# sebrahimi1988/dss-ml-at-scale

Measured on AMD Instinct MI355X. Metric: samples/sec, higher is better.
Workload: dtype bf16; 1 GPU; model=resnet18, global_batch=212, parallelism=dp1+hipgraph

## Files before the change

### mi355x_scale/models/resnet.py

```python
from __future__ import annotations

from typing import List, Optional, Type, Union

import torch
import torch.nn as nn

from ..ops.conv3x3 import Conv3x3
from ..ops.fused_bn import FusedBNReLU2d
from ..ops.maxpool import MaxPool3x3s2
from ..ops.stemconv import StemConv2d


def _conv3x3(cin: int, cout: int, stride: int = 1) -> nn.Conv2d:
    if stride == 1 and cin == cout:
        return Conv3x3(cin, cout)
    return nn.Conv2d(cin, cout, 3, stride=stride, padding=1, bias=False)


def _conv1x1(cin: int, cout: int, stride: int = 1) -> nn.Conv2d:
    return nn.Conv2d(cin, cout, 1, stride=stride, bias=False)


class BasicBlock(nn.Module):
    expansion = 1

    def __init__(self, cin: int, cout: int, stride: int = 1,
                 downsample: Optional[nn.Module] = None):
        super().__init__()
        self.conv1 = _conv3x3(cin, cout, stride)
        self.bn1 = FusedBNReLU2d(cout)
        self.conv2 = _conv3x3(cout, cout)
        self.bn2 = FusedBNReLU2d(cout)
        self.downsample = downsample

    def forward(self, x: torch.Tensor) -> torch.Tensor:
        identity = x if self.downsample is None else self.downsample(x)
        out = self.bn1(self.conv1(x))
        return self.bn2(self.conv2(out), residual=identity)


class Bottleneck(nn.Module):
    expansion = 4

    def __init__(self, cin: int, cout: int, stride: int = 1,
                 downsample: Optional[nn.Module] = None):
        super().__init__()
        self.conv1 = _conv1x1(cin, cout)
        self.bn1 = FusedBNReLU2d(cout)
        self.conv2 = _conv3x3(cout, cout, stride)
        self.bn2 = FusedBNReLU2d(cout)
        self.conv3 = _conv1x1(cout, cout * self.expansion)
        self.bn3 = FusedBNReLU2d(cout * self.expansion)
        self.downsample = downsample

    def forward(self, x: torch.Tensor) -> torch.Tensor:
        identity = x if self.downsample is None else self.downsample(x)
        out = self.bn1(self.conv1(x))
        out = self.bn2(self.conv2(out))
        return self.bn3(self.conv3(out), residual=identity)


class ResNet(nn.Module):
    def __init__(self, block: Type[Union[BasicBlock, Bottleneck]],
                 layers: List[int], num_classes: int = 1000,
                 zero_init_residual: bool = True):
        super().__init__()
        self.inplanes = 64
        self.conv1 = StemConv2d()
        self.bn1 = FusedBNReLU2d(64)
        self.maxpool = MaxPool3x3s2()
        self.layer1 = self._make_layer(block, 64, layers[0])
        self.layer2 = self._make_layer(block, 128, layers[1], stride=2)
        self.layer3 = self._make_layer(block, 256, layers[2], stride=2)
        self.layer4 = self._make_layer(block, 512, layers[3], stride=2)
        self.avgpool = nn.AdaptiveAvgPool2d(1)
        self.fc = nn.Linear(512 * block.expansion, num_classes)

        for m in self.modules():
            if isinstance(m, nn.Conv2d):
                nn.init.kaiming_normal_(m.weight, mode="fan_out",
                                        nonlinearity="relu")
            elif isinstance(m, nn.BatchNorm2d):
                nn.init.ones_(m.weight)
                nn.init.zeros_(m.bias)
        if zero_init_residual:
            for m in self.modules():
                if isinstance(m, Bottleneck):
                    nn.init.zeros_(m.bn3.weight)
                elif isinstance(m, BasicBlock):
                    nn.init.zeros_(m.bn2.weight)

    def _make_layer(self, block, planes: int, blocks: int,
                    stride: int = 1) -> nn.Sequential:
        downsample = None
        if stride != 1 or self.inplanes != planes * block.expansion:
            downsample = nn.Sequential(
                _conv1x1(self.inplanes, planes * block.expansion, stride),
                FusedBNReLU2d(planes * block.expansion, relu=False),
            )
        layers = [block(self.inplanes, planes, stride, downsample)]
        self.inplanes = planes * block.expansion
        layers += [block(self.inplanes, planes) for _ in range(1, blocks)]
        return nn.Sequential(*layers)

    def forward(self, x: torch.Tensor) -> torch.Tensor:
        if self.bn1.training and self.conv1.stats_ok(x):
            x, partial = self.conv1.forward_with_stats(x)
            x = self.bn1.forward_pooled(x, partial)
        else:
            x = self.bn1.forward_pooled(self.conv1(x))
        x = self.layer4(self.layer3(self.layer2(self.layer1(x))))
        x = self.avgpool(x).flatten(1)
        return self.fc(x)


def resnet18(num_classes: int = 1000) -> ResNet:
    return ResNet(BasicBlock, [2, 2, 2, 2], num_classes)


def resnet34(num_classes: int = 1000) -> ResNet:
    return ResNet(BasicBlock, [3, 4, 6, 3], num_classes)


def resnet50(num_classes: int = 1000) -> ResNet:
    return ResNet(Bottleneck, [3, 4, 6, 3], num_classes)


MODELS = {"resnet18": resnet18, "resnet34": resnet34, "resnet50": resnet50}


def build_model(name: str, num_classes: int = 1000) -> ResNet:
    try:
        return MODELS[name](num_classes)
    except KeyError:
        raise ValueError(f"unknown model {name!r}; have {sorted(MODELS)}")
```

### mi355x_scale/ops/csrc/bindings.cpp

```cpp

#include <torch/extension.h>
#include <ATen/hip/HIPContext.h>
#include <hip/hip_runtime.h>

extern "C" void launch_normalize_u8_to_bf16(
    const uint8_t* in, void* out, const float* scale_dev,
    const float* shift_dev, long long n, hipStream_t stream);

void normalize_u8_to_bf16(torch::Tensor in, torch::Tensor out,
                          torch::Tensor scale, torch::Tensor shift) {
  TORCH_CHECK(in.is_cuda() && out.is_cuda(), "tensors must be on GPU");
  TORCH_CHECK(in.scalar_type() == torch::kUInt8, "input must be uint8");
  TORCH_CHECK(out.scalar_type() == torch::kBFloat16, "output must be bf16");
  TORCH_CHECK(in.is_contiguous(), "input must be contiguous (NHWC)");
  TORCH_CHECK(in.numel() == out.numel(), "element count mismatch");
  TORCH_CHECK(scale.is_cuda() && shift.is_cuda() && scale.numel() == 3 &&
                  shift.numel() == 3,
              "scale/shift must be 3-element device float tensors");
  TORCH_CHECK(scale.scalar_type() == torch::kFloat32 &&
              shift.scalar_type() == torch::kFloat32,
              "scale/shift must be float32");
  auto stream = at::cuda::getCurrentHIPStream();
  launch_normalize_u8_to_bf16(
      in.data_ptr<uint8_t>(), out.data_ptr(),
// ... 81 lines not shown

void groupfit_final(torch::Tensor yT, torch::Tensor xc0, torch::Tensor xc1,
                    torch::Tensor xc2, torch::Tensor pj0, torch::Tensor pj1,
                    torch::Tensor pj2, torch::Tensor best_order,
                    torch::Tensor fitted, torch::Tensor params,
                    torch::Tensor status,
                    torch::Tensor b0, torch::Tensor b1, torch::Tensor b2,
                    torch::Tensor w0, torch::Tensor w1, torch::Tensor w2) {
  _check_f32(yT, "yT"); _check_f32(fitted, "fitted");
  _check_f32(params, "params");
  TORCH_CHECK(best_order.scalar_type() == torch::kInt32 &&
              best_order.is_cuda());
  int T = yT.size(0);
  long long G = yT.size(1);
  TORCH_CHECK(fitted.size(0) == T && fitted.size(1) == G);
  auto stream = at::cuda::getCurrentHIPStream();
  auto fp = [](torch::Tensor& t) -> const float* {
    return t.numel() ? t.data_ptr<float>() : nullptr;
  };
  launch_groupfit_final(
      yT.data_ptr<float>(), xc0.data_ptr<float>(), xc1.data_ptr<float>(),
      xc2.data_ptr<float>(), pj0.data_ptr<float>(), pj1.data_ptr<float>(),
      pj2.data_ptr<float>(), best_order.data_ptr<int>(),
      fitted.data_ptr<float>(), params.data_ptr<float>(),
      status.data_ptr<uint8_t>(),
      fp(b0), fp(b1), fp(b2), fp(w0), fp(w1), fp(w2),
      T, G, (int)xc0.size(1), stream.stream());
}

void diff_center(torch::Tensor yT, torch::Tensor wc, torch::Tensor wm,
                 int64_t S, int64_t d) {
  _check_f32(yT, "yT"); _check_f32(wc, "wc"); _check_f32(wm, "wm");
  auto stream = at::cuda::getCurrentHIPStream();
  launch_diff_center(yT.data_ptr<float>(), wc.data_ptr<float>(),
                     wm.data_ptr<float>(), yT.size(0), yT.size(1),
                     (int)S, (int)d, stream.stream());
}

void exog_project_mfma(torch::Tensor P, torch::Tensor wc,
                       torch::Tensor beta) {
  _check_f32(P, "P"); _check_f32(wc, "wc"); _check_f32(beta, "beta");
  TORCH_CHECK(P.size(1) == wc.size(0), "K mismatch");
  TORCH_CHECK(beta.size(0) == P.size(0) && beta.size(1) == wc.size(1));
  TORCH_CHECK(P.size(0) <= 16, "KX must fit one MFMA row tile");
  auto stream = at::cuda::getCurrentHIPStream();
  launch_exog_project_mfma(P.data_ptr<float>(), wc.data_ptr<float>(),
                           beta.data_ptr<float>(), P.size(1), wc.size(1),
                           P.size(0), stream.stream());
}


extern "C" int bn_reduce_blocks(long long rows, int C);
extern "C" void launch_bn_fwd_reduce(const void* x, float* partial,
                                     int nblocks, long long rows, int C,
                                     hipStream_t stream);
extern "C" void launch_bn_fwd_finalize(const float* partial, int nblocks,
                                       float* mean, float* invstd,
                                       float* running_mean,
                                       float* running_var, float momentum,
                                       float eps, long long rows, int C,
                                       int update_running,
                                       long long* num_batches_tracked,
                                       hipStream_t stream);
extern "C" void launch_bn_pool_bwd_reduce(
    const void* dp, const unsigned char* code, const void* x,
    const float* mean, const float* invstd, const float* weight,
    const float* bias, float* partial, int nblocks, int N, int H, int W,
    int Ho, int Wo, int C, hipStream_t stream);
extern "C" void launch_bn_pool_bwd_apply(
    const void* dp, const unsigned char* code, const void* x,
    const float* mean, const float* invstd, const float* bias,
    const float* k, void* dx, int N, int H, int W, int Ho, int Wo, int C,
    hipStream_t stream);
extern "C" void launch_bn_fwd_apply(const void* x, const void* res, void* y,
                                    const float* mean, const float* invstd,
                                    const float* weight, const float* bias,
                                    long long rows, int C, int relu,
                                    hipStream_t stream);
extern "C" void launch_bn_bwd_reduce(const void* dz, const void* y,
                                     const void* x, const float* mean,
                                     const float* invstd, float* partial,
                                     void* dym, int nblocks, long long rows,
                                     int C, int relu, hipStream_t stream);
extern "C" void launch_bn_bwd_reduce_rm(const void* dz, const void* x,
                                        const float* mean,
                                        const float* invstd,
                                        const float* weight,
                                        const float* bias, float* partial,
                                        void* dym, int nblocks,
                                        long long rows, int C,
                                        hipStream_t stream);
extern "C" void launch_bn_bwd_apply_rm(const void* dz, const void* x,
                                       const float* mean,
                                       const float* invstd,
                                       const float* bias, const float* k,
                                       void* dx, long long rows, int C,
                                       hipStream_t stream);
extern "C" void launch_bn_bwd_apply_dym(const void* dym, const void* x,
                                        const float* mean,
                                        const float* invstd, const float* k,
                                        void* dx, long long rows, int C,
                                        hipStream_t stream);
extern "C" void launch_bn_bwd_finalize(const float* partial, int nblocks,
                                       const float* invstd,
                                       const float* weight, float* dweight,
                                       float* dbias, float* k, long long rows,
                                       int C, int accumulate,
                                       hipStream_t stream);
extern "C" void launch_bn_bwd_apply(const void* dz, const void* y,
                                    const void* x, const float* mean,
                                    const float* invstd, const float* k,
                                    void* dx, void* dres, long long rows,
                                    int C, int relu, hipStream_t stream);

static void _check_bn_act(const torch::Tensor& t, const char* name) {
  TORCH_CHECK(t.is_cuda() && t.scalar_type() == torch::kBFloat16,
              name, " must be bf16 on GPU");
}

static long long _bn_rows(const torch::Tensor& x, int64_t C) {
  TORCH_CHECK(C % 8 == 0 && 256 % (C / 8) == 0,
              "C must be 8*2^k and <= 2048, got ", C);
  TORCH_CHECK(x.numel() % C == 0, "numel not divisible by C");
  return (long long)(x.numel() / C);
}

torch::Tensor bn_fwd_reduce(torch::Tensor x, int64_t C) {
  _check_bn_act(x, "x");
  long long rows = _bn_rows(x, C);
  int nb = bn_reduce_blocks(rows, (int)C);
  auto partial = torch::empty(
      {(int64_t)nb * 2 * C},
      torch::TensorOptions().dtype(torch::kFloat32).device(x.device()));
  launch_bn_fwd_reduce(x.data_ptr(), partial.data_ptr<float>(), nb, rows,
                       (int)C, at::cuda::getCurrentHIPStream().stream());
  return partial;
}

void bn_fwd_finalize(torch::Tensor partial, torch::Tensor mean,
                     torch::Tensor invstd, torch::Tensor running_mean,
                     torch::Tensor running_var, double momentum, double eps,
                     int64_t rows, int64_t C, bool update_running,
                     c10::optional<torch::Tensor> num_batches_tracked) {
  _check_f32(partial, "partial"); _check_f32(mean, "mean");
  _check_f32(invstd, "invstd");
  _check_f32(running_mean, "running_mean");
  _check_f32(running_var, "running_var");
  TORCH_CHECK(partial.numel() % (2 * C) == 0, "partial must be [nb*2C]");
  int nb = (int)(partial.numel() / (2 * C));
  long long* nbt_p = nullptr;
  if (num_batches_tracked.has_value()) {
    const torch::Tensor& nbt = *num_batches_tracked;
    TORCH_CHECK(nbt.is_cuda() && nbt.scalar_type() == torch::kInt64 &&
                    nbt.numel() == 1,
                "num_batches_tracked must be a 1-element int64 GPU tensor");
    nbt_p = reinterpret_cast<long long*>(nbt.data_ptr<int64_t>());
  }
  launch_bn_fwd_finalize(partial.data_ptr<float>(), nb,
                         mean.data_ptr<float>(), invstd.data_ptr<float>(),
                         running_mean.data_ptr<float>(),
                         running_var.data_ptr<float>(), (float)momentum,
                         (float)eps, rows, (int)C, update_running ? 1 : 0,
                         nbt_p, at::cuda::getCurrentHIPStream().stream());
}

void bn_fwd_apply(torch::Tensor x, torch::Tensor res, torch::Tensor y,
                  torch::Tensor mean, torch::Tensor invstd,
                  torch::Tensor weight, torch::Tensor bias, int64_t C,
                  bool relu) {
  _check_bn_act(x, "x"); _check_bn_act(y, "y");
  _check_f32(mean, "mean"); _check_f32(invstd, "invstd");
  _check_f32(weight, "weight"); _check_f32(bias, "bias");
  const void* res_p = nullptr;
  if (res.defined() && res.numel()) {
    _check_bn_act(res, "res");
    TORCH_CHECK(res.numel() == x.numel(), "residual shape mismatch");
    res_p = res.data_ptr();
  }
  launch_bn_fwd_apply(x.data_ptr(), res_p, y.data_ptr(),
                      mean.data_ptr<float>(), invstd.data_ptr<float>(),
                      weight.data_ptr<float>(), bias.data_ptr<float>(),
                      _bn_rows(x, C), (int)C, relu ? 1 : 0,
                      at::cuda::getCurrentHIPStream().stream());
}

torch::Tensor bn_bwd_reduce(torch::Tensor dz, torch::Tensor y,
                            torch::Tensor x, torch::Tensor mean,
                            torch::Tensor invstd, torch::Tensor dym,
                            int64_t C, bool relu) {
  _check_bn_act(dz, "dz"); _check_bn_act(y, "y"); _check_bn_act(x, "x");
  void* dym_p = nullptr;
  if (dym.defined() && dym.numel()) {
    _check_bn_act(dym, "dym");
    TORCH_CHECK(dym.numel() == x.numel(), "dym shape mismatch");
    dym_p = dym.data_ptr();
  }
  long long rows = _bn_rows(x, C);
  int nb = bn_reduce_blocks(rows, (int)C);
  auto partial = torch::empty(
      {(int64_t)nb * 2 * C},
      torch::TensorOptions().dtype(torch::kFloat32).device(x.device()));
  launch_bn_bwd_reduce(dz.data_ptr(), y.data_ptr(), x.data_ptr(),
                       mean.data_ptr<float>(), invstd.data_ptr<float>(),
                       partial.data_ptr<float>(), dym_p, nb, rows, (int)C,
                       relu ? 1 : 0,
                       at::cuda::getCurrentHIPStream().stream());
  return partial;
}

torch::Tensor bn_bwd_reduce_rm(torch::Tensor dz, torch::Tensor x,
                               torch::Tensor mean, torch::Tensor invstd,
                               torch::Tensor weight, torch::Tensor bias,
                               torch::Tensor dym, int64_t C) {
  _check_bn_act(dz, "dz"); _check_bn_act(x, "x");
  _check_f32(mean, "mean"); _check_f32(invstd, "invstd");
  _check_f32(weight, "weight"); _check_f32(bias, "bias");
  void* dym_p = nullptr;
  if (dym.defined() && dym.numel()) {
    _check_bn_act(dym, "dym");
    TORCH_CHECK(dym.numel() == x.numel(), "dym shape mismatch");
    dym_p = dym.data_ptr();
  }
  long long rows = _bn_rows(x, C);
  int nb = bn_reduce_blocks(rows, (int)C);
  auto partial = torch::empty(
      {(int64_t)nb * 2 * C},
      torch::TensorOptions().dtype(torch::kFloat32).device(x.device()));
  launch_bn_bwd_reduce_rm(dz.data_ptr(), x.data_ptr(),
                          mean.data_ptr<float>(), invstd.data_ptr<float>(),
                          weight.data_ptr<float>(), bias.data_ptr<float>(),
                          partial.data_ptr<float>(), dym_p, nb, rows,
                          (int)C, at::cuda::getCurrentHIPStream().stream());
  return partial;
}

void bn_bwd_apply_rm(torch::Tensor dz, torch::Tensor x, torch::Tensor mean,
                     torch::Tensor invstd, torch::Tensor bias,
                     torch::Tensor k, torch::Tensor dx, int64_t C) {
  _check_bn_act(dz, "dz"); _check_bn_act(x, "x"); _check_bn_act(dx, "dx");
  _check_f32(mean, "mean"); _check_f32(invstd, "invstd");
  _check_f32(bias, "bias"); _check_f32(k, "k");
  launch_bn_bwd_apply_rm(dz.data_ptr(), x.data_ptr(),
                         mean.data_ptr<float>(), invstd.data_ptr<float>(),
                         bias.data_ptr<float>(), k.data_ptr<float>(),
                         dx.data_ptr(), _bn_rows(x, C), (int)C,
                         at::cuda::getCurrentHIPStream().stream());
}

void bn_bwd_apply_dym(torch::Tensor dym, torch::Tensor x,
                      torch::Tensor mean, torch::Tensor invstd,
                      torch::Tensor k, torch::Tensor dx, int64_t C) {
  _check_bn_act(dym, "dym"); _check_bn_act(x, "x"); _check_bn_act(dx, "dx");
  _check_f32(mean, "mean"); _check_f32(invstd, "invstd");
  _check_f32(k, "k");
  launch_bn_bwd_apply_dym(dym.data_ptr(), x.data_ptr(),
                          mean.data_ptr<float>(), invstd.data_ptr<float>(),
                          k.data_ptr<float>(), dx.data_ptr(),
                          _bn_rows(x, C), (int)C,
                          at::cuda::getCurrentHIPStream().stream());
}

void bn_bwd_finalize(torch::Tensor partial, torch::Tensor invstd,
                     torch::Tensor weight, torch::Tensor dweight,
                     torch::Tensor dbias, torch::Tensor k, int64_t rows,
                     int64_t C, bool accumulate) {
  _check_f32(partial, "partial"); _check_f32(invstd, "invstd");
  _check_f32(weight, "weight"); _check_f32(dweight, "dweight");
  _check_f32(dbias, "dbias"); _check_f32(k, "k");
  TORCH_CHECK(k.numel() == 3 * C, "k must be [3C]");
  TORCH_CHECK(partial.numel() % (2 * C) == 0, "partial must be [nb*2C]");
  int nb = (int)(partial.numel() / (2 * C));
  launch_bn_bwd_finalize(partial.data_ptr<float>(), nb,
                         invstd.data_ptr<float>(),
                         weight.data_ptr<float>(), dweight.data_ptr<float>(),
                         dbias.data_ptr<float>(), k.data_ptr<float>(), rows,
                         (int)C, accumulate ? 1 : 0,
                         at::cuda::getCurrentHIPStream().stream());
}

void bn_bwd_apply(torch::Tensor dz, torch::Tensor y, torch::Tensor x,
                  torch::Tensor mean, torch::Tensor invstd, torch::Tensor k,
                  torch::Tensor dx, torch::Tensor dres, int64_t C,
                  bool relu) {
  _check_bn_act(dz, "dz"); _check_bn_act(y, "y"); _check_bn_act(x, "x");
  _check_bn_act(dx, "dx");
  _check_f32(mean, "mean"); _check_f32(invstd, "invstd");
  _check_f32(k, "k");
  void* dres_p = nullptr;
  if (dres.defined() && dres.numel()) {
// ... 259 lines not shown
                   torch::Tensor dw, int64_t phase_mask = 7) {
  TORCH_CHECK(x.is_cuda() && x.scalar_type() == torch::kBFloat16);
  TORCH_CHECK(dy.is_cuda() && dy.scalar_type() == torch::kBFloat16);
  TORCH_CHECK(dw_f32.scalar_type() == torch::kFloat32 &&
              dw_f32.numel() == 64 * 160);
  TORCH_CHECK(dw.scalar_type() == torch::kBFloat16 &&
              dw.numel() == 64 * 7 * 7 * 3);
  int Nb = x.size(0), H = x.size(1), W = x.size(2);
  int HO = dy.size(1), WO = dy.size(2);
  launch_stem_conv_wrw(x.data_ptr(), dy.data_ptr(),
                       dw_f32.data_ptr<float>(), dw.data_ptr(),
                       Nb, H, W, HO, WO,
                       at::cuda::getCurrentHIPStream().stream(),
                       (int)phase_mask);
}

void conv3x3_wrw(torch::Tensor x, torch::Tensor dy, torch::Tensor part,
                 torch::Tensor dw, int64_t phase_mask = 7,
                 int64_t chunks = 0) {
  TORCH_CHECK(x.is_cuda() && x.scalar_type() == torch::kBFloat16);
  TORCH_CHECK(dy.is_cuda() && dy.scalar_type() == torch::kBFloat16);
  int Nb = x.size(0), H = x.size(1), W = x.size(2), C = x.size(3);
  TORCH_CHECK(dy.size(1) == H && dy.size(2) == W && dy.size(3) == C,
              "same-shape 3x3 s1 conv only");
  TORCH_CHECK(C % 64 == 0 && C <= 2048, "C must be a multiple of 64");
  TORCH_CHECK(W >= 3 && W <= 64, "row length outside kernel bounds");
  const int nch = conv3x3_wrw_chunks(Nb, H, C, (int)chunks);
  TORCH_CHECK(part.scalar_type() == torch::kFloat32 &&
              part.numel() >= (long long)nch * C * 9 * C,
              "partial buffer too small for ", nch, " chunks");
  TORCH_CHECK(dw.scalar_type() == torch::kBFloat16 &&
              dw.numel() == (long long)C * 9 * C);
  launch_conv3x3_wrw(x.data_ptr(), dy.data_ptr(), part.data_ptr<float>(),
                     dw.data_ptr(), Nb, H, W, C, nch,
                     at::cuda::getCurrentHIPStream().stream(),
                     (int)phase_mask);
}

int64_t conv3x3_wrw_nchunks(int64_t Nb, int64_t H, int64_t C,
                            int64_t chunks) {
  return conv3x3_wrw_chunks((int)Nb, (int)H, (int)C, (int)chunks);
}

PYBIND11_MODULE(TORCH_EXTENSION_NAME, m) {
  m.def("conv3x3_wrw", &conv3x3_wrw,
        "MFMA 3x3/s1 CxC weight grad (fp32 accum, bf16 cast to view)",
        pybind11::arg("x"), pybind11::arg("dy"), pybind11::arg("part"),
        pybind11::arg("dw"), pybind11::arg("phase_mask") = 7,
        pybind11::arg("chunks") = 0);
  m.def("conv3x3_wrw_nchunks", &conv3x3_wrw_nchunks,
        "partial-buffer chunk count the wrw launcher will use");
  m.def("stem_conv_fwd", &stem_conv_fwd,
        "MFMA stem conv fwd (7x7 s2, 3->64, NHWC bf16)",
        pybind11::arg("x"), pybind11::arg("w"), pybind11::arg("out"),
        pybind11::arg("wp_scratch"), pybind11::arg("phase_mask") = 7,
        pybind11::arg("partial") = pybind11::none());
  m.def("stem_fwd_blocks", &stem_fwd_blocks,
        "block (= BN partial slot) count of the fused-statistics stem fwd");
  m.def("stem_conv_wrw", &stem_conv_wrw,
        "MFMA stem conv weight-grad (fp32 accum + bf16 cast)",
        pybind11::arg("x"), pybind11::arg("dy"), pybind11::arg("dw_f32"),
        pybind11::arg("dw"), pybind11::arg("phase_mask") = 7);
  m.def("normalize_u8_to_bf16", &normalize_u8_to_bf16,
        "fused uint8 NHWC -> normalized bf16 (same memory order)");
  m.def("groupfit_eval", &groupfit_eval,
        "batched per-group ARIMAX candidate evaluation (validation MSE)");
  m.def("groupfit_final", &groupfit_final,
        "batched per-group final fit (fitted values + params)");
  m.def("diff_center", &diff_center,
        "difference + per-group centering of the time-major panel");
  m.def("exog_project_mfma", &exog_project_mfma,
        "design-matrix GEMM beta = P @ Wc on f32 MFMA");
  m.def("bn_fwd_reduce", &bn_fwd_reduce);
  m.def("bn_fwd_finalize", &bn_fwd_finalize,
        "mean/invstd + running stats (+ optional int64 step counter)",
        pybind11::arg("partial"), pybind11::arg("mean"),
        pybind11::arg("invstd"), pybind11::arg("running_mean"),
        pybind11::arg("running_var"), pybind11::arg("momentum"),
        pybind11::arg("eps"), pybind11::arg("rows"), pybind11::arg("C"),
        pybind11::arg("update_running"),
        pybind11::arg("num_batches_tracked") = pybind11::none());
  m.def("bn_fwd_apply", &bn_fwd_apply);
  m.def("bn_bwd_reduce", &bn_bwd_reduce);
  m.def("bn_bwd_reduce_rm", &bn_bwd_reduce_rm);
  m.def("bn_bwd_apply_rm", &bn_bwd_apply_rm);
  m.def("bn_bwd_finalize", &bn_bwd_finalize);
  m.def("bn_bwd_apply", &bn_bwd_apply);
  m.def("bn_bwd_apply_dym", &bn_bwd_apply_dym);
  m.def("adam_step", &adam_step,
        "fused flat Adam step (one kernel over p/g/m/v)");
  m.def("maxpool3x3s2_fwd", &maxpool3x3s2_fwd);
  m.def("bn_maxpool3x3s2_fwd", &bn_maxpool3x3s2_fwd);
  m.def("maxpool3x3s2_bwd", &maxpool3x3s2_bwd);
  m.def("bn_pool_bwd_reduce", &bn_pool_bwd_reduce,
        "stem BN bwd reduce with the max-unpool rebuilt in registers");
  m.def("bn_pool_bwd_apply", &bn_pool_bwd_apply,
        "stem BN bwd apply with the max-unpool rebuilt in registers");
  m.def("adam_step_mixed", &adam_step_mixed,
        "fused flat Adam with bf16 params/grads + fp32 master");
  m.def("arma_generate", &arma_generate,
        "batched ARMA(p,q) sample paths, one group per lane");
}
```

### mi355x_scale/ops/csrc/fused_bn.hip

```cpp

#include <hip/hip_runtime.h>
#include <hip/hip_bf16.h>

typedef __hip_bfloat16 bf16;

#define VEC 8

union BVec {
  uint4 u;
  bf16 h[VEC];
};

static __device__ __forceinline__ BVec load8(const bf16* p) {
  BVec v;
  v.u = *reinterpret_cast<const uint4*>(p);
  return v;
}

static __device__ __forceinline__ void store8(bf16* p, const BVec& v) {
  *reinterpret_cast<uint4*>(p) = v.u;
}

__global__ __launch_bounds__(256) void bn_fwd_reduce_kernel(
    const bf16* __restrict__ x, float* __restrict__ partial,
// ... 155 lines not shown
    const long long off = row * C + (long long)lane * VEC;
    BVec v = load8(x + off);
    BVec r;
    if (RES) r = load8(res + off);
    BVec o;
#pragma unroll
    for (int j = 0; j < VEC; ++j) {
      float f = fmaf(__bfloat162float(v.h[j]), a[j], b[j]);
      if (RES) f += __bfloat162float(r.h[j]);
      if (RELU) f = fmaxf(f, 0.f);
      o.h[j] = __float2bfloat16(f);
    }
    store8(y + off, o);
  }
}

template <bool RELU, bool WRITE_DY>
__global__ __launch_bounds__(256) void bn_bwd_reduce_kernel(
    const bf16* __restrict__ dz, const bf16* __restrict__ y,
    const bf16* __restrict__ x, const float* __restrict__ mean,
    const float* __restrict__ invstd, float* __restrict__ partial,
    bf16* __restrict__ dym, long long rows, int C) {
  const int lanes = C / VEC;
  const int lane = threadIdx.x % lanes;
  const int rsub = threadIdx.x / lanes;
  const int rows_per_iter = blockDim.x / lanes;
  const long long rstride = (long long)gridDim.x * rows_per_iter;

  float m[VEC], is[VEC];
#pragma unroll
  for (int j = 0; j < VEC; ++j) {
    int c = lane * VEC + j;
    m[j] = mean[c];
    is[j] = invstd[c];
  }

  float sdy[VEC] = {0.f}, sdyx[VEC] = {0.f};
  for (long long row = (long long)blockIdx.x * rows_per_iter + rsub;
       row < rows; row += rstride) {
    const long long off = row * C + (long long)lane * VEC;
    BVec g = load8(dz + off);
    BVec xv = load8(x + off);
    BVec yv;
    if (RELU) yv = load8(y + off);
    BVec dyv;
#pragma unroll
    for (int j = 0; j < VEC; ++j) {
      float dy = __bfloat162float(g.h[j]);
      if (RELU && __bfloat162float(yv.h[j]) <= 0.f) dy = 0.f;
      float xhat = (__bfloat162float(xv.h[j]) - m[j]) * is[j];
      sdy[j] += dy;
      sdyx[j] += dy * xhat;
      if (WRITE_DY) dyv.h[j] = __float2bfloat16(dy);
    }
    if (WRITE_DY) store8(dym + off, dyv);
  }

  __shared__ float lds[256 * 2 * VEC];
  float* mys = &lds[(rsub * lanes + lane) * 2 * VEC];
#pragma unroll
  for (int j = 0; j < VEC; ++j) {
    mys[j] = sdy[j];
    mys[VEC + j] = sdyx[j];
  }
  __syncthreads();
  for (int step = rows_per_iter >> 1; step > 0; step >>= 1) {
    if (rsub < step) {
      const float* other = &lds[((rsub + step) * lanes + lane) * 2 * VEC];
#pragma unroll
      for (int j = 0; j < 2 * VEC; ++j) mys[j] += other[j];
    }
    __syncthreads();
  }
  if (rsub == 0) {
#pragma unroll
    for (int j = 0; j < VEC; ++j) {
      partial[(long long)(lane * VEC + j) * gridDim.x + blockIdx.x] = mys[j];
      partial[(long long)(C + lane * VEC + j) * gridDim.x + blockIdx.x] =
          mys[VEC + j];
    }
  }
}

__global__ __launch_bounds__(256) void bn_bwd_finalize_kernel(
    const float* __restrict__ partial, int nblocks,
    const float* __restrict__ invstd, const float* __restrict__ weight,
    float* __restrict__ dweight, float* __restrict__ dbias,
    float* __restrict__ k, long long rows, int C, int accumulate) {
  int c = blockIdx.x * (blockDim.x / 64) + threadIdx.x / 64;
  int lane = threadIdx.x % 64;
  if (c >= C) return;
  float sdy = 0.f, sdyx = 0.f;
  for (int b = lane; b < nblocks; b += 64) {
    sdy += partial[(long long)c * nblocks + b];
    sdyx += partial[(long long)(C + c) * nblocks + b];
  }
#pragma unroll
  for (int off = 32; off > 0; off >>= 1) {
    sdy += __shfl_down(sdy, off, 64);
    sdyx += __shfl_down(sdyx, off, 64);
  }
  if (lane != 0) return;
  dbias[c] = accumulate ? dbias[c] + sdy : sdy;
  dweight[c] = accumulate ? dweight[c] + sdyx : sdyx;
  k[c] = weight[c] * invstd[c];
  k[C + c] = sdy / (float)rows;
  k[2 * C + c] = sdyx / (float)rows;
}

__global__ __launch_bounds__(256) void bn_bwd_apply_dym_kernel(
    const bf16* __restrict__ dym, const bf16* __restrict__ x,
    const float* __restrict__ mean, const float* __restrict__ invstd,
    const float* __restrict__ k, bf16* __restrict__ dx, long long rows,
    int C) {
  const int lanes = C / VEC;
  const int lane = threadIdx.x % lanes;
  const int rsub = threadIdx.x / lanes;
  const int rows_per_iter = blockDim.x / lanes;
  const long long rstride = (long long)gridDim.x * rows_per_iter;

  float m[VEC], is[VEC], wv[VEC], k1[VEC], k2[VEC];
#pragma unroll
  for (int j = 0; j < VEC; ++j) {
    int c = lane * VEC + j;
    m[j] = mean[c];
    is[j] = invstd[c];
    wv[j] = k[c];
    k1[j] = k[C + c];
    k2[j] = k[2 * C + c];
  }

  for (long long row = (long long)blockIdx.x * rows_per_iter + rsub;
       row < rows; row += rstride) {
    const long long off = row * C + (long long)lane * VEC;
    BVec g = load8(dym + off);
    BVec xv = load8(x + off);
    BVec odx;
#pragma unroll
    for (int j = 0; j < VEC; ++j) {
      float dy = __bfloat162float(g.h[j]);
      float xhat = (__bfloat162float(xv.h[j]) - m[j]) * is[j];
      odx.h[j] = __float2bfloat16(wv[j] * (dy - k1[j] - xhat * k2[j]));
    }
    store8(dx + off, odx);
  }
}

template <bool RELU, bool RES>
__global__ __launch_bounds__(256) void bn_bwd_apply_kernel(
    const bf16* __restrict__ dz, const bf16* __restrict__ y,
    const bf16* __restrict__ x, const float* __restrict__ mean,
    const float* __restrict__ invstd, const float* __restrict__ k,
    bf16* __restrict__ dx, bf16* __restrict__ dres, long long rows, int C) {
  const int lanes = C / VEC;
  const int lane = threadIdx.x % lanes;
  const int rsub = threadIdx.x / lanes;
  const int rows_per_iter = blockDim.x / lanes;
  const long long rstride = (long long)gridDim.x * rows_per_iter;

  float m[VEC], is[VEC], wv[VEC], k1[VEC], k2[VEC];
#pragma unroll
  for (int j = 0; j < VEC; ++j) {
    int c = lane * VEC + j;
    m[j] = mean[c];
    is[j] = invstd[c];
    wv[j] = k[c];
// ... 332 lines not shown
        odx.h[j] = __float2bfloat16(v);
      }
      store8(dx + t.pix[p], odx);
    }
  }
}


static int pick_grid(long long rows, int C) {
  int rows_per_iter = 256 / (C / VEC);
  long long blocks = (rows + rows_per_iter - 1) / rows_per_iter;
  if (blocks > 2080) blocks = 2080;
  return (int)(blocks > 0 ? blocks : 1);
}

extern "C" int bn_reduce_blocks(long long rows, int C) {
  int rows_per_iter = 256 / (C / VEC);
  long long blocks = (rows + rows_per_iter - 1) / rows_per_iter;
  if (blocks > 512) blocks = 512;
  return (int)(blocks > 0 ? blocks : 1);
}

extern "C" void launch_bn_fwd_reduce(const void* x, float* partial,
                                     int nblocks, long long rows, int C,
                                     hipStream_t stream) {
  hipLaunchKernelGGL(bn_fwd_reduce_kernel, dim3(nblocks), dim3(256), 0,
                     stream, (const bf16*)x, partial, rows, C);
}

#define BN_FINALIZE_WIDE_MIN 1024

extern "C" void launch_bn_fwd_finalize(const float* partial, int nblocks,
                                       float* mean, float* invstd,
                                       float* running_mean,
                                       float* running_var, float momentum,
                                       float eps, long long rows, int C,
                                       int update_running,
                                       long long* num_batches_tracked,
                                       hipStream_t stream) {
  if (nblocks > BN_FINALIZE_WIDE_MIN) {
    hipLaunchKernelGGL(bn_fwd_finalize_wide_kernel, dim3(C), dim3(256), 0,
                       stream, partial, nblocks, mean, invstd, running_mean,
                       running_var, momentum, eps, rows, C, update_running,
                       num_batches_tracked);
    return;
  }
  hipLaunchKernelGGL(bn_fwd_finalize_kernel, dim3((C + 3) / 4),
                     dim3(256), 0, stream, partial, nblocks, mean, invstd,
                     running_mean, running_var, momentum, eps, rows, C,
                     update_running, num_batches_tracked);
}

extern "C" void launch_bn_fwd_apply(const void* x, const void* res, void* y,
                                    const float* mean, const float* invstd,
                                    const float* weight, const float* bias,
                                    long long rows, int C, int relu,
                                    hipStream_t stream) {
  dim3 grid(pick_grid(rows, C)), block(256);
#define APPLY(R, S)                                                       \
  hipLaunchKernelGGL((bn_fwd_apply_kernel<R, S>), grid, block, 0, stream, \
                     (const bf16*)x, (const bf16*)res, (bf16*)y, mean,    \
                     invstd, weight, bias, rows, C)
  if (relu && res) APPLY(true, true);
  else if (relu) APPLY(true, false);
  else if (res) APPLY(false, true);
  else APPLY(false, false);
#undef APPLY
}

extern "C" void launch_bn_bwd_reduce(const void* dz, const void* y,
                                     const void* x, const float* mean,
                                     const float* invstd, float* partial,
                                     void* dym, int nblocks, long long rows,
                                     int C, int relu, hipStream_t stream) {
  dim3 grid(nblocks), block(256);
#define REDUCE(R, W)                                                       \
  hipLaunchKernelGGL((bn_bwd_reduce_kernel<R, W>), grid, block, 0, stream, \
                     (const bf16*)dz, (const bf16*)y, (const bf16*)x,      \
                     mean, invstd, partial, (bf16*)dym, rows, C)
  if (relu && dym) REDUCE(true, true);
  else if (relu) REDUCE(true, false);
  else if (dym) REDUCE(false, true);
  else REDUCE(false, false);
#undef REDUCE
}

extern "C" void launch_bn_bwd_reduce_rm(const void* dz, const void* x,
                                        const float* mean,
                                        const float* invstd,
                                        const float* weight,
                                        const float* bias, float* partial,
                                        void* dym, int nblocks,
                                        long long rows, int C,
                                        hipStream_t stream) {
  dim3 grid(nblocks), block(256);
  if (dym)
    hipLaunchKernelGGL((bn_bwd_reduce_rm_kernel<true>), grid, block, 0,
                       stream, (const bf16*)dz, (const bf16*)x, mean,
                       invstd, weight, bias, partial, (bf16*)dym, rows, C);
  else
    hipLaunchKernelGGL((bn_bwd_reduce_rm_kernel<false>), grid, block, 0,
                       stream, (const bf16*)dz, (const bf16*)x, mean,
                       invstd, weight, bias, partial, nullptr, rows, C);
}

extern "C" void launch_bn_bwd_apply_rm(const void* dz, const void* x,
                                       const float* mean,
                                       const float* invstd,
                                       const float* bias, const float* k,
                                       void* dx, long long rows, int C,
                                       hipStream_t stream) {
  hipLaunchKernelGGL(bn_bwd_apply_rm_kernel, dim3(pick_grid(rows, C)),
                     dim3(256), 0, stream, (const bf16*)dz,
                     (const bf16*)x, mean, invstd, bias, k, (bf16*)dx,
                     rows, C);
}

extern "C" void launch_bn_pool_bwd_reduce(
    const void* dp, const unsigned char* code, const void* x,
    const float* mean, const float* invstd, const float* weight,
    const float* bias, float* partial, int nblocks, int N, int H, int W,
    int Ho, int Wo, int C, hipStream_t stream) {
  hipLaunchKernelGGL(bn_pool_bwd_reduce_kernel, dim3(nblocks), dim3(256), 0,
                     stream, (const bf16*)dp, code, (const bf16*)x, mean,
                     invstd, weight, bias, partial, N, H, W, Ho, Wo, C);
}

extern "C" void launch_bn_pool_bwd_apply(
    const void* dp, const unsigned char* code, const void* x,
    const float* mean, const float* invstd, const float* bias,
    const float* k, void* dx, int N, int H, int W, int Ho, int Wo, int C,
    hipStream_t stream) {
  hipLaunchKernelGGL(bn_pool_bwd_apply_kernel,
                     dim3(pick_grid((long long)N * Ho * Wo, C)), dim3(256),
                     0, stream, (const bf16*)dp, code, (const bf16*)x, mean,
                     invstd, bias, k, (bf16*)dx, N, H, W, Ho, Wo, C);
}

extern "C" void launch_bn_bwd_apply_dym(const void* dym, const void* x,
                                        const float* mean,
                                        const float* invstd, const float* k,
                                        void* dx, long long rows, int C,
                                        hipStream_t stream) {
  hipLaunchKernelGGL(bn_bwd_apply_dym_kernel, dim3(pick_grid(rows, C)),
                     dim3(256), 0, stream, (const bf16*)dym, (const bf16*)x,
                     mean, invstd, k, (bf16*)dx, rows, C);
}

extern "C" void launch_bn_bwd_finalize(const float* partial, int nblocks,
                                       const float* invstd,
                                       const float* weight, float* dweight,
                                       float* dbias, float* k, long long rows,
                                       int C, int accumulate,
                                       hipStream_t stream) {
  hipLaunchKernelGGL(bn_bwd_finalize_kernel, dim3((C + 3) / 4),
                     dim3(256), 0, stream, partial, nblocks, invstd, weight,
                     dweight, dbias, k, rows, C, accumulate);
}

extern "C" void launch_bn_bwd_apply(const void* dz, const void* y,
                                    const void* x, const float* mean,
                                    const float* invstd, const float* k,
                                    void* dx, void* dres, long long rows,
                                    int C, int relu, hipStream_t stream) {
  dim3 grid(pick_grid(rows, C)), block(256);
#define APPLY(R, S)                                                        \
// ... 10 lines not shown
```

### mi355x_scale/ops/fused_bn.py

```python
from __future__ import annotations

from typing import Optional

import torch
import torch.nn as nn
import torch.nn.functional as F

from . import _C, require_ext


def _hip_supported(x: torch.Tensor) -> bool:
    c = x.shape[1]
    return (x.is_cuda and x.dtype == torch.bfloat16 and x.dim() == 4
            and c % 8 == 0 and c <= 2048 and (256 % (c // 8)) == 0)


class _FusedBNFn(torch.autograd.Function):
    @staticmethod
    def forward(ctx, x, residual, weight, bias, running_mean, running_var,
                momentum, eps, relu, num_batches_tracked):
        C = x.shape[1]
        rows = x.numel() // C
        dev = x.device
        mean = torch.empty(C, dtype=torch.float32, device=dev)
        invstd = torch.empty(C, dtype=torch.float32, device=dev)
        partial = _C.bn_fwd_reduce(x, C)
        _C.bn_fwd_finalize(partial, mean, invstd, running_mean, running_var,
                           momentum, eps, rows, C, True, num_batches_tracked)
        y = torch.empty_like(x)
        res = residual if residual is not None else x.new_empty(0)
        _C.bn_fwd_apply(x, res, y, mean, invstd, weight, bias, C, relu)
        ctx.save_for_backward(x, y if residual is not None else x,
                              mean, invstd, weight, bias)
        ctx.relu = relu
        ctx.has_res = residual is not None
        return y

    @staticmethod
    def backward(ctx, dz):
        x, y, mean, invstd, weight, bias = ctx.saved_tensors
        C = x.shape[1]
        rows = x.numel() // C
        dev = x.device
        if not dz.is_contiguous(memory_format=torch.channels_last):
            dz = dz.contiguous(memory_format=torch.channels_last)
        k = torch.empty(3 * C, dtype=torch.float32, device=dev)
        def _grad_view(p):
            g = p.grad
            if (g is not None and g.is_cuda and g.is_contiguous()
                    and g.dtype == torch.float32 and g.numel() == C):
                return g
            return None

        import os
        wg, bg = _grad_view(weight), _grad_view(bias)
        fuse_acc = (torch.cuda.is_current_stream_capturing()
                    and wg is not None and bg is not None
                    and os.environ.get("MI355X_BN_FUSED_ACC", "1") == "1")
        if fuse_acc:
            dweight, dbias = wg, bg
        else:
            dweight = torch.empty(C, dtype=torch.float32, device=dev)
            dbias = torch.empty(C, dtype=torch.float32, device=dev)
        dx = torch.empty_like(x)
        if ctx.has_res:
            dym = torch.empty_like(x)
            partial = _C.bn_bwd_reduce(dz, y, x, mean, invstd, dym, C,
                                       ctx.relu)
            _C.bn_bwd_finalize(partial, invstd, weight, dweight, dbias, k,
                               rows, C, fuse_acc)
            _C.bn_bwd_apply_dym(dym, x, mean, invstd, k, dx, C)
            return (dx, dym, None if fuse_acc else dweight,
                    None if fuse_acc else dbias, None, None, None, None,
                    None, None)
        if ctx.relu:
            partial = _C.bn_bwd_reduce_rm(dz, x, mean, invstd, weight,
                                          bias, x.new_empty(0), C)
            _C.bn_bwd_finalize(partial, invstd, weight, dweight, dbias, k,
                               rows, C, fuse_acc)
            _C.bn_bwd_apply_rm(dz, x, mean, invstd, bias, k, dx, C)
        else:
            partial = _C.bn_bwd_reduce(dz, y, x, mean, invstd,
                                       x.new_empty(0), C, False)
            _C.bn_bwd_finalize(partial, invstd, weight, dweight, dbias, k,
                               rows, C, fuse_acc)
            _C.bn_bwd_apply(dz, y, x, mean, invstd, k, dx, x.new_empty(0),
                            C, False)
        return (dx, None, None if fuse_acc else dweight,
                None if fuse_acc else dbias, None, None, None, None, None,
                None)


class _FusedBNPoolFn(torch.autograd.Function):

    @staticmethod
    def forward(ctx, x, weight, bias, running_mean, running_var,
                momentum, eps, training, num_batches_tracked, partial=None):
        C = x.shape[1]
        dev = x.device
        if training:
            rows = x.numel() // C
            mean = torch.empty(C, dtype=torch.float32, device=dev)
            invstd = torch.empty(C, dtype=torch.float32, device=dev)
            if partial is None:
                partial = _C.bn_fwd_reduce(x, C)
            _C.bn_fwd_finalize(partial, mean, invstd, running_mean,
                               running_var, momentum, eps, rows, C, True,
                               num_batches_tracked)
        else:
            mean = running_mean.to(torch.float32)
            invstd = torch.rsqrt(running_var.to(torch.float32) + eps)
        n, _, h, w = x.shape
        ho, wo = (h + 1) // 2, (w + 1) // 2
        y = torch.empty((n, C, ho, wo), dtype=x.dtype, device=dev,
                        memory_format=torch.channels_last)
        code = torch.empty(n * ho * wo * C, dtype=torch.uint8, device=dev)
        _C.bn_maxpool3x3s2_fwd(x, mean, invstd, weight, bias, y, code)
        ctx.save_for_backward(x, mean, invstd, weight, bias, code)
        return y

    @staticmethod
    def backward(ctx, dp):
        x, mean, invstd, weight, bias, code = ctx.saved_tensors
        C = x.shape[1]
        rows = x.numel() // C
        dev = x.device
        if not dp.is_contiguous(memory_format=torch.channels_last):
            dp = dp.contiguous(memory_format=torch.channels_last)
        import os
        fused_unpool = os.environ.get("MI355X_BN_POOL_FUSED_BWD", "1") != "0"
        k = torch.empty(3 * C, dtype=torch.float32, device=dev)

        def _grad_view(p):
            g = p.grad
            if (g is not None and g.is_cuda and g.is_contiguous()
                    and g.dtype == torch.float32 and g.numel() == C):
                return g
            return None

        wg, bg = _grad_view(weight), _grad_view(bias)
        fuse_acc = (torch.cuda.is_current_stream_capturing()
                    and wg is not None and bg is not None
                    and os.environ.get("MI355X_BN_FUSED_ACC", "1") == "1")
        if fuse_acc:
            dweight, dbias = wg, bg
        else:
            dweight = torch.empty(C, dtype=torch.float32, device=dev)
            dbias = torch.empty(C, dtype=torch.float32, device=dev)
        dx = torch.empty_like(x)
        if fused_unpool:
            partial = _C.bn_pool_bwd_reduce(dp, code, x, mean, invstd,
                                            weight, bias)
            _C.bn_bwd_finalize(partial, invstd, weight, dweight, dbias, k,
                               rows, C, fuse_acc)
            _C.bn_pool_bwd_apply(dp, code, x, mean, invstd, bias, k, dx)
        else:
            dz = torch.empty_like(x)
            _C.maxpool3x3s2_bwd(dp, code, dz)
            partial = _C.bn_bwd_reduce_rm(dz, x, mean, invstd, weight, bias,
                                          x.new_empty(0), C)
            _C.bn_bwd_finalize(partial, invstd, weight, dweight, dbias, k,
                               rows, C, fuse_acc)
            _C.bn_bwd_apply_rm(dz, x, mean, invstd, bias, k, dx, C)
        return (dx, None if fuse_acc else dweight,
                None if fuse_acc else dbias, None, None, None, None, None,
                None, None)


class FusedBNReLU2d(nn.Module):

    gpu_fallbacks: list = []

    def __init__(self, num_features: int, eps: float = 1e-5,
                 momentum: float = 0.1, relu: bool = True):
        super().__init__()
        self.num_features = num_features
        self.eps = eps
        self.momentum = momentum
        self.relu = relu
        self.weight = nn.Parameter(torch.ones(num_features))
        self.bias = nn.Parameter(torch.zeros(num_features))
        self.register_buffer("running_mean", torch.zeros(num_features))
        self.register_buffer("running_var", torch.ones(num_features))
        self.register_buffer("num_batches_tracked",
                             torch.tensor(0, dtype=torch.long))

    def extra_repr(self) -> str:
        return (f"{self.num_features}, eps={self.eps}, "
                f"momentum={self.momentum}, relu={self.relu}")

    def forward_pooled(self, x: torch.Tensor,
                       partial: Optional[torch.Tensor] = None
                       ) -> torch.Tensor:
        assert self.relu, "pooled fusion is relu-only"
        if _hip_supported(x):
            require_ext()
            x = x.contiguous(memory_format=torch.channels_last)
            return _FusedBNPoolFn.apply(
                x, self.weight, self.bias, self.running_mean,
                self.running_var, self.momentum, self.eps, self.training,
                self.num_batches_tracked,
                partial if self.training else None)
        return F.max_pool2d(self.forward(x), 3, stride=2, padding=1)

    def forward(self, x: torch.Tensor,
                residual: Optional[torch.Tensor] = None) -> torch.Tensor:
        if _hip_supported(x):
            require_ext()
            x = x.contiguous(memory_format=torch.channels_last)
            if residual is not None:
                residual = residual.contiguous(
                    memory_format=torch.channels_last)
            if self.training:
                return _FusedBNFn.apply(
                    x, residual, self.weight, self.bias, self.running_mean,
                    self.running_var, self.momentum, self.eps, self.relu,
                    self.num_batches_tracked)
            if not (torch.is_grad_enabled() and
                    (x.requires_grad or self.weight.requires_grad)):
                invstd = torch.rsqrt(self.running_var + self.eps)
                y = torch.empty_like(x)
                res = (residual if residual is not None else x.new_empty(0))
                _C.bn_fwd_apply(x, res, y, self.running_mean, invstd,
                                self.weight, self.bias, x.shape[1],
                                self.relu)
                return y
        if self.training:
            self.num_batches_tracked += 1
        if x.is_cuda and len(FusedBNReLU2d.gpu_fallbacks) < 256:
            FusedBNReLU2d.gpu_fallbacks.append(
                (tuple(x.shape), str(x.dtype), self.training))
        y = F.batch_norm(x, self.running_mean, self.running_var, self.weight,
                         self.bias, self.training, self.momentum, self.eps)
        if residual is not None:
            y = y + residual
        return F.relu(y) if self.relu else y
```

Measured before the change: 27020 samples/s.

## Fuse residual-branch gradient accumulation into BN backward reduce via twin outputs

The residual BN forward now returns two outputs, the activation and an alias of it. The next block uses the alias for its conv path and the twin for its skip path, so autograd delivers two separate gradients to the BN backward instead of summing them in a separate add kernel. A new join reduce kernel loads both gradients, sums them in bf16, applies the ReLU mask and accumulates the BN statistics in one pass. This removes an elementwise add and a full activation read/write per block, at the cost of a more fragile autograd path that relies on attaching a tensor attribute.

```diff
diff --git a/mi355x_scale/models/resnet.py b/mi355x_scale/models/resnet.py
--- a/mi355x_scale/models/resnet.py
+++ b/mi355x_scale/models/resnet.py
@@ -21,6 +21,11 @@
     return nn.Conv2d(cin, cout, 1, stride=stride, bias=False)
 
 
+def _join_twin(x: torch.Tensor) -> torch.Tensor:
+    twin = getattr(x, FusedBNReLU2d.JOIN_ATTR, None)
+    return x if twin is None else twin
+
+
 class BasicBlock(nn.Module):
     expansion = 1
 
@@ -34,7 +39,8 @@
         self.downsample = downsample
 
     def forward(self, x: torch.Tensor) -> torch.Tensor:
-        identity = x if self.downsample is None else self.downsample(x)
+        skip = _join_twin(x)
+        identity = skip if self.downsample is None else self.downsample(skip)
         out = self.bn1(self.conv1(x))
         return self.bn2(self.conv2(out), residual=identity)
 
@@ -54,7 +60,8 @@
         self.downsample = downsample
 
     def forward(self, x: torch.Tensor) -> torch.Tensor:
-        identity = x if self.downsample is None else self.downsample(x)
+        skip = _join_twin(x)
+        identity = skip if self.downsample is None else self.downsample(skip)
         out = self.bn1(self.conv1(x))
         out = self.bn2(self.conv2(out))
         return self.bn3(self.conv3(out), residual=identity)
diff --git a/mi355x_scale/ops/csrc/bindings.cpp b/mi355x_scale/ops/csrc/bindings.cpp
--- a/mi355x_scale/ops/csrc/bindings.cpp
+++ b/mi355x_scale/ops/csrc/bindings.cpp
@@ -187,6 +187,13 @@
                                      const float* invstd, float* partial,
                                      void* dym, int nblocks, long long rows,
                                      int C, int relu, hipStream_t stream);
+extern "C" void launch_bn_bwd_reduce_join(const void* dz1, const void* dz2,
+                                          const void* y, const void* x,
+                                          const float* mean,
+                                          const float* invstd,
+                                          float* partial, void* dym,
+                                          int nblocks, long long rows, int C,
+                                          int relu, hipStream_t stream);
 extern "C" void launch_bn_bwd_reduce_rm(const void* dz, const void* x,
                                         const float* mean,
                                         const float* invstd,
@@ -310,6 +317,38 @@
                        partial.data_ptr<float>(), dym_p, nb, rows, (int)C,
                        relu ? 1 : 0,
                        at::cuda::getCurrentHIPStream().stream());
+  return partial;
+}
+
+torch::Tensor bn_bwd_reduce_join(torch::Tensor dz1, torch::Tensor dz2,
+                                 torch::Tensor y, torch::Tensor x,
+                                 torch::Tensor mean, torch::Tensor invstd,
+                                 torch::Tensor dym, int64_t C, bool relu) {
+  _check_bn_act(dz1, "dz1"); _check_bn_act(dz2, "dz2");
+  _check_bn_act(y, "y"); _check_bn_act(x, "x"); _check_bn_act(dym, "dym");
+  _check_f32(mean, "mean"); _check_f32(invstd, "invstd");
+  TORCH_CHECK(mean.numel() == C && invstd.numel() == C,
+              "mean/invstd must have C elements");
+  TORCH_CHECK(x.dim() == 4 && x.size(1) == C &&
+                  x.is_contiguous(at::MemoryFormat::ChannelsLast),
+              "x must be a channels_last [N,C,H,W] tensor");
+  const torch::Tensor* maps[] = {&dz1, &dz2, &y, &dym};
+  const char* names[] = {"dz1", "dz2", "y", "dym"};
+  for (int i = 0; i < 4; ++i)
+    TORCH_CHECK(maps[i]->sizes() == x.sizes() &&
+                    maps[i]->is_contiguous(at::MemoryFormat::ChannelsLast),
+                names[i], " must match x (channels_last)");
+  long long rows = _bn_rows(x, C);
+  int nb = bn_reduce_blocks(rows, (int)C);
+  auto partial = torch::empty(
+      {(int64_t)nb * 2 * C},
+      torch::TensorOptions().dtype(torch::kFloat32).device(x.device()));
+  launch_bn_bwd_reduce_join(dz1.data_ptr(), dz2.data_ptr(), y.data_ptr(),
+                            x.data_ptr(), mean.data_ptr<float>(),
+                            invstd.data_ptr<float>(),
+                            partial.data_ptr<float>(), dym.data_ptr(), nb,
+                            rows, (int)C, relu ? 1 : 0,
+                            at::cuda::getCurrentHIPStream().stream());
   return partial;
 }
 
@@ -735,6 +774,7 @@
         pybind11::arg("num_batches_tracked") = pybind11::none());
   m.def("bn_fwd_apply", &bn_fwd_apply);
   m.def("bn_bwd_reduce", &bn_bwd_reduce);
+  m.def("bn_bwd_reduce_join", &bn_bwd_reduce_join);
   m.def("bn_bwd_reduce_rm", &bn_bwd_reduce_rm);
   m.def("bn_bwd_apply_rm", &bn_bwd_apply_rm);
   m.def("bn_bwd_finalize", &bn_bwd_finalize);
diff --git a/mi355x_scale/ops/csrc/fused_bn.hip b/mi355x_scale/ops/csrc/fused_bn.hip
--- a/mi355x_scale/ops/csrc/fused_bn.hip
+++ b/mi355x_scale/ops/csrc/fused_bn.hip
@@ -261,6 +261,76 @@
   }
 }
 
+template <bool RELU>
+__global__ __launch_bounds__(256) void bn_bwd_reduce_join_kernel(
+    const bf16* __restrict__ dz1, const bf16* __restrict__ dz2,
+    const bf16* __restrict__ y, const bf16* __restrict__ x,
+    const float* __restrict__ mean, const float* __restrict__ invstd,
+    float* __restrict__ partial, bf16* __restrict__ dym, long long rows,
+    int C) {
+  const int lanes = C / VEC;
+  const int lane = threadIdx.x % lanes;
+  const int rsub = threadIdx.x / lanes;
+  const int rows_per_iter = blockDim.x / lanes;
+  const long long rstride = (long long)gridDim.x * rows_per_iter;
+
+  float m[VEC], is[VEC];
+#pragma unroll
+  for (int j = 0; j < VEC; ++j) {
+    int c = lane * VEC + j;
+    m[j] = mean[c];
+    is[j] = invstd[c];
+  }
+
+  float sdy[VEC] = {0.f}, sdyx[VEC] = {0.f};
+  for (long long row = (long long)blockIdx.x * rows_per_iter + rsub;
+       row < rows; row += rstride) {
+    const long long off = row * C + (long long)lane * VEC;
+    BVec g1 = load8(dz1 + off);
+    BVec g2 = load8(dz2 + off);
+    BVec xv = load8(x + off);
+    BVec yv;
+    if (RELU) yv = load8(y + off);
+    BVec dyv;
+#pragma unroll
+    for (int j = 0; j < VEC; ++j) {
+      float dy = __bfloat162float(__float2bfloat16(
+          __bfloat162float(g1.h[j]) + __bfloat162float(g2.h[j])));
+      if (RELU && __bfloat162float(yv.h[j]) <= 0.f) dy = 0.f;
+      float xhat = (__bfloat162float(xv.h[j]) - m[j]) * is[j];
+      sdy[j] += dy;
+      sdyx[j] += dy * xhat;
+      dyv.h[j] = __float2bfloat16(dy);
+    }
+    store8(dym + off, dyv);
+  }
+
+  __shared__ float lds[256 * 2 * VEC];
+  float* mys = &lds[(rsub * lanes + lane) * 2 * VEC];
+#pragma unroll
+  for (int j = 0; j < VEC; ++j) {
+    mys[j] = sdy[j];
+    mys[VEC + j] = sdyx[j];
+  }
+  __syncthreads();
+  for (int step = rows_per_iter >> 1; step > 0; step >>= 1) {
+    if (rsub < step) {
+      const float* other = &lds[((rsub + step) * lanes + lane) * 2 * VEC];
+#pragma unroll
+      for (int j = 0; j < 2 * VEC; ++j) mys[j] += other[j];
+    }
+    __syncthreads();
+  }
+  if (rsub == 0) {
+#pragma unroll
+    for (int j = 0; j < VEC; ++j) {
+      partial[(long long)(lane * VEC + j) * gridDim.x + blockIdx.x] = mys[j];
+      partial[(long long)(C + lane * VEC + j) * gridDim.x + blockIdx.x] =
+          mys[VEC + j];
+    }
+  }
+}
+
 __global__ __launch_bounds__(256) void bn_bwd_finalize_kernel(
     const float* __restrict__ partial, int nblocks,
     const float* __restrict__ invstd, const float* __restrict__ weight,
@@ -759,6 +829,24 @@
   else if (relu) REDUCE(true, false);
   else if (dym) REDUCE(false, true);
   else REDUCE(false, false);
+#undef REDUCE
+}
+
+extern "C" void launch_bn_bwd_reduce_join(const void* dz1, const void* dz2,
+                                          const void* y, const void* x,
+                                          const float* mean,
+                                          const float* invstd,
+                                          float* partial, void* dym,
+                                          int nblocks, long long rows, int C,
+                                          int relu, hipStream_t stream) {
+  dim3 grid(nblocks), block(256);
+#define REDUCE(R)                                                         \
+  hipLaunchKernelGGL((bn_bwd_reduce_join_kernel<R>), grid, block, 0,      \
+                     stream, (const bf16*)dz1, (const bf16*)dz2,          \
+                     (const bf16*)y, (const bf16*)x, mean, invstd,        \
+                     partial, (bf16*)dym, rows, C)
+  if (relu) REDUCE(true);
+  else REDUCE(false);
 #undef REDUCE
 }
 
diff --git a/mi355x_scale/ops/fused_bn.py b/mi355x_scale/ops/fused_bn.py
--- a/mi355x_scale/ops/fused_bn.py
+++ b/mi355x_scale/ops/fused_bn.py
@@ -1,5 +1,6 @@
 from __future__ import annotations
 
+import os
 from typing import Optional
 
 import torch
@@ -18,7 +19,7 @@
 class _FusedBNFn(torch.autograd.Function):
     @staticmethod
     def forward(ctx, x, residual, weight, bias, running_mean, running_var,
-                momentum, eps, relu, num_batches_tracked):
+                momentum, eps, relu, num_batches_tracked, join=False):
         C = x.shape[1]
         rows = x.numel() // C
         dev = x.device
@@ -34,16 +35,26 @@
                               mean, invstd, weight, bias)
         ctx.relu = relu
         ctx.has_res = residual is not None
-        return y
-
-    @staticmethod
-    def backward(ctx, dz):
+        if not join:
+            return y
+        ctx.set_materialize_grads(False)
+        return y, y.view_as(y)
+
+    @staticmethod
+    def backward(ctx, dz, dz2=None):
         x, y, mean, invstd, weight, bias = ctx.saved_tensors
         C = x.shape[1]
         rows = x.numel() // C
         dev = x.device
+        if dz is None:
+            dz, dz2 = dz2, None
+        if dz is None:
+            return (None,) * 11
         if not dz.is_contiguous(memory_format=torch.channels_last):
             dz = dz.contiguous(memory_format=torch.channels_last)
+        if (dz2 is not None and
+                not dz2.is_contiguous(memory_format=torch.channels_last)):
+            dz2 = dz2.contiguous(memory_format=torch.channels_last)
         k = torch.empty(3 * C, dtype=torch.float32, device=dev)
         def _grad_view(p):
             g = p.grad
@@ -65,14 +76,20 @@
         dx = torch.empty_like(x)
         if ctx.has_res:
             dym = torch.empty_like(x)
-            partial = _C.bn_bwd_reduce(dz, y, x, mean, invstd, dym, C,
-                                       ctx.relu)
+            if dz2 is not None:
+                partial = _C.bn_bwd_reduce_join(dz, dz2, y, x, mean, invstd,
+                                                dym, C, ctx.relu)
+                FusedBNReLU2d.join_calls += 1
+            else:
+                partial = _C.bn_bwd_reduce(dz, y, x, mean, invstd, dym, C,
+                                           ctx.relu)
             _C.bn_bwd_finalize(partial, invstd, weight, dweight, dbias, k,
                                rows, C, fuse_acc)
             _C.bn_bwd_apply_dym(dym, x, mean, invstd, k, dx, C)
             return (dx, dym, None if fuse_acc else dweight,
                     None if fuse_acc else dbias, None, None, None, None,
-                    None, None)
+                    None, None, None)
+        assert dz2 is None
         if ctx.relu:
             partial = _C.bn_bwd_reduce_rm(dz, x, mean, invstd, weight,
                                           bias, x.new_empty(0), C)
@@ -88,7 +105,7 @@
                             C, False)
         return (dx, None, None if fuse_acc else dweight,
                 None if fuse_acc else dbias, None, None, None, None, None,
-                None)
+                None, None)
 
 
 class _FusedBNPoolFn(torch.autograd.Function):
@@ -170,6 +187,10 @@
 class FusedBNReLU2d(nn.Module):
 
     gpu_fallbacks: list = []
+
+    join_calls: int = 0
+
+    JOIN_ATTR = "_bn_join_twin"
 
     def __init__(self, num_features: int, eps: float = 1e-5,
                  momentum: float = 0.1, relu: bool = True):
@@ -212,10 +233,17 @@
                 residual = residual.contiguous(
                     memory_format=torch.channels_last)
             if self.training:
-                return _FusedBNFn.apply(
+                join = (residual is not None and
+                        os.environ.get("MI355X_BN_JOIN", "1") != "0")
+                out = _FusedBNFn.apply(
                     x, residual, self.weight, self.bias, self.running_mean,
                     self.running_var, self.momentum, self.eps, self.relu,
-                    self.num_batches_tracked)
+                    self.num_batches_tracked, join)
+                if not join:
+                    return out
+                y, alias = out
+                setattr(alias, FusedBNReLU2d.JOIN_ATTR, y)
+                return alias
             if not (torch.is_grad_enabled() and
                     (x.requires_grad or self.weight.requires_grad)):
                 invstd = torch.rsqrt(self.running_var + self.eps)
```

Result: faster. 27290 samples/s, median of 6 (+1.0%).
